# LucaAmbrogioni/Brancher

Measured on AMD Instinct MI355X. Metric: ELBO iters/sec at num_samples=300 per GPU (300-sample-equivalent iterations, whole job), higher is better.
Workload: dtype f32

## Files before the change

brancher_amd/csrc/spec_main.h:

```cpp
#pragma once

namespace bsvi {

#if defined(__HIP_DEVICE_COMPILE__)
#define SPEC_CONST_AS __attribute__((address_space(4)))
#define SPEC_RELOAD_ARGS() asm volatile("" : "+s"(ka))
#else
#define SPEC_CONST_AS
#define SPEC_RELOAD_ARGS()
#endif

#define SPEC_TAB_PTR (4 * SPEC_N_UNIFORM)
#define SPEC_TAB_POS (SPEC_TAB_PTR + SPEC_N_PARAMS + 1)
#define SPEC_TAB_IDX (SPEC_TAB_POS + SPEC_N_POS)
#define SPEC_TAB_MASK (SPEC_TAB_IDX + SPEC_N_POS)

__device__ __forceinline__ void spec_lds_barrier() {
#if defined(__HIP_DEVICE_COMPILE__)
    asm volatile("s_waitcnt lgkmcnt(0)\n\ts_barrier" ::: "memory");
#endif
}

__device__ __noinline__ float spec_utransform_rare(uint32_t t, float x) { return utransform((int)t, x); }
__device__ __noinline__ float spec_utransform_grad_rare(uint32_t t, float x) { return utransform_grad((int)t, x); }
// ... 298 lines not shown
    const uint32_t oid = tid - own_base;
    bool own_fast = false;
#if SPEC_DRAW_OWNERS
    SpecOwn own = {};
#endif
    if (oid < SPEC_N_PARAMS) {
        const uint32_t j0 = TAB[SPEC_TAB_PTR + oid], j1 = TAB[SPEC_TAB_PTR + oid + 1];
        if (j1 - j0 <= 2u) {
            own_fast = true;
#if !SPEC_DRAW_OWNERS
            SpecOwn own;
#endif
            own.n = j1 - j0;
            own.mask = 0;
            own.theta = PS[oid];
            own.s0 = own.s1 = own.s2 = own.st = 0.0f;
            own.p1 = own.p2 = 1.0;
            own.a[0] = own.a[1] = own.b[0] = own.b[1] = 0.0f;
            own.pos[0] = own.pos[1] = own.k[0] = own.k[1] = own.tr[0] = own.tr[1] = 0;
            if (step) {
                own.s0 = PS[SPEC_NP_PAD + oid]; own.s1 = PS[2 * SPEC_NP_PAD + oid];
                own.s2 = PS[3 * SPEC_NP_PAD + oid]; own.st = PS[4 * SPEC_NP_PAD + oid];
                own.mask = TAB[SPEC_TAB_MASK + oid];
                const bsvi_opt_cfg cfg0 = SPEC_A->cfg;
                if (cfg0.kind != BSVI_OPT_SGD && own.st != 0.0f) {
                    own.p1 = pow((double)cfg0.beta1, (double)own.st);
                    own.p2 = pow((double)cfg0.beta2, (double)own.st);
                }
            }
#pragma unroll
            for (uint32_t e = 0; e < 2u; ++e) {
                if (e < own.n) {
                    const uint32_t k = TAB[SPEC_TAB_IDX + j0 + e];
                    own.pos[e] = TAB[SPEC_TAB_POS + j0 + e];
                    own.k[e] = k;
                    own.tr[e] = TAB[4 * k + 1] & 0xFFu;
                    own.a[e] = __uint_as_float(TAB[4 * k + 2]);
                    own.b[e] = __uint_as_float(TAB[4 * k + 3]);
                }
            }
#if !SPEC_DRAW_OWNERS
            spec_own_store(OWN + 5 * oid, own);
#endif
        }
    }

    SPEC_RELOAD_ARGS();
    SpecBody B0;
    B0.n_local = SPEC_A->n_local;
    B0.seed_lo = SPEC_A->seed_lo;
    B0.seed_hi = SPEC_A->seed_hi;
#if SPEC_DIAG
    B0.noise = SPEC_A->noise;
    B0.samples_out = SPEC_A->samples_out;
    B0.noise_out = SPEC_A->noise_out;
    B0.fvalue_out = SPEC_A->fvalue_out;
    B0.f_weight = SPEC_A->f_weight;
    B0.q_weight = SPEC_A->q_weight;
#else
    B0.noise = nullptr; B0.samples_out = nullptr; B0.noise_out = nullptr; B0.fvalue_out = nullptr;
    B0.f_weight = nullptr; B0.q_weight = nullptr;
#endif
    unsigned long long off0 = ((unsigned long long)SPEC_A->offset_hi << 32) | SPEC_A->offset_lo;
    if (const unsigned long long* const offset_dev = SPEC_A->offset_dev) off0 += *offset_dev;
    const uint32_t n_global = SPEC_A->n_global;
    const uint32_t pretraining = SPEC_A->pretraining_iterations;
#if SPEC_ACCUMULATE_CHUNKS
#define SPEC_LOOP_MANY 1
#define SPEC_GEN_OVER 0x7fff0000u
    const unsigned int gen0 = 0;
    if (G > 1 && mode == SPEC_MODE_LOOP && blockIdx.x != 0 &&
        __hip_atomic_load(SPEC_A->ticket + 64, __ATOMIC_RELAXED, __HIP_MEMORY_SCOPE_AGENT) >= SPEC_GEN_OVER) return;
#else
#define SPEC_LOOP_MANY 0
#endif
#if SPEC_EXCHANGE
    uint32_t xseq0 = 0;
    if (const SpecExchange* const xg0 = SPEC_A->xchg) xseq0 = reinterpret_cast<const uint32_t*>(xg0->peer[xg0->rank])[XCHG_CALLS_WORD + 1];
#endif

#if defined(SPEC_DEBUG_STAMPS)
    unsigned long long stamp[12] = {0, 0, 0, 0, 0, 0, 0, 0, 0, 0, 0, 0};
#define SPEC_STAMP(i) if (it == n_it / 2) stamp[i] = __builtin_amdgcn_s_memtime()
    unsigned long long rstamp[6] = {0, 0, 0, 0, 0, 0};
#define SPEC_RSTAMP(i) if (it == n_it / 2) rstamp[i] = __builtin_amdgcn_s_memtime()
#define SPEC_RSTAMP_NEXT() if (it == n_it / 2 + 1u) rstamp[5] = __builtin_amdgcn_s_memtime()
#define SPEC_RSTAMP_WRITE()                                                                                              \
    if (lane == 0u && SPEC_A->loss_slot && n_it > 16u + 8u * SPEC_MAX_WAVES) {                                           \
        asm volatile("s_waitcnt vmcnt(0)" ::: "memory");                                                                 \
        for (int i = 1; i < 6; ++i) SPEC_A->loss_slot[16u + 8u * wave + i] = (float)(rstamp[i] - rstamp[0]);               \
        SPEC_A->loss_slot[16u + 8u * wave] = 1.0f;                                                                       \
    }
#else
#define SPEC_STAMP(i)
#define SPEC_RSTAMP(i)
#define SPEC_RSTAMP_NEXT()
#define SPEC_RSTAMP_WRITE()
#endif
#if SPEC_KEEP_NOISE && !SPEC_DIAG && !SPEC_ACCUMULATE_CHUNKS && !defined(SPEC_DEBUG_NO_DRAW) && !defined(SPEC_NO_EARLY_DRAW)
#define SPEC_EARLY_DRAW 1
    SpecNoise Z;
    bool noise_ready = false;
#else
#define SPEC_EARLY_DRAW 0
#endif
#if SPEC_DRAW_WAVE
    if (draw_service && draw_wave) {
        if (lane == 0u) { RED[8 + 2 * wave] = 0.0f; RED[9 + 2 * wave] = 0.0f; }
        const uint32_t n_draw = W - WSN, k = wave - WSN;
        const uint32_t first = k;
        uint32_t before = 0;
        for (uint32_t j = 0; j < k; ++j) before += (((WSN + j) & 3u) != 1u) ? 1u : 0u;
        const uint32_t second = n_draw + before;
        const bool has_first = first < WSN, has_second = (wave & 3u) != 1u && second < WSN;
        auto draw_for = [&](uint32_t target, unsigned long long offn, SpecNoise& Zd) {
            SpecLane Tn = T;
            Tn.n = target * 64u + lane;
            Tn.active = Tn.n < B0.n_local;
            Tn.nc = Tn.active ? Tn.n : (B0.n_local - 1u);
            Tn.nidx = sample_base + Tn.nc;
            Tn.off_lo = (uint32_t)offn;
            Tn.off_hi = (uint32_t)(offn >> 32);
            Tn.vz = T.vz;
            spec_draw(B0, Tn, Zd);
        };
#if SPEC_DRAW_OWNERS
        (void)has_first; (void)has_second;
        const uint32_t kown = own_wave - WSN, n_other = n_draw - 1u, rest = WSN - 1u;
        const uint32_t j = k < kown ? k : k - 1u, per = rest / n_other, extra = rest % n_other;
        const uint32_t set_a = __builtin_amdgcn_readfirstlane(1u + j * per + (j < extra ? j : extra));
        const uint32_t n_sets = __builtin_amdgcn_readfirstlane(per + (j < extra ? 1u : 0u));
        const bool owners = __builtin_amdgcn_readfirstlane(wave == own_wave ? 1 : 0) != 0;
        for (uint32_t it = 0; it < n_it; ++it) {
            const bool more = it + 1u < n_it, last = !more;
            spec_lds_barrier();
            SPEC_RSTAMP(0);
            SPEC_RSTAMP_NEXT();
            SpecNoise Za, Zb;
            float fac[2] = {0.0f, 0.0f};
            AdamBias bias = {1.0, 1.0, 0.0f, 0.0f};
            if (owners) {
                SPEC_RELOAD_ARGS();
                const bsvi_opt_cfg cfg = SPEC_A->cfg;
#pragma unroll
                for (uint32_t e = 0; e < 2u; ++e) fac[e] = own.b[e] * spec_utransform_grad(own.tr[e], own.theta);
                if (cfg.kind != BSVI_OPT_SGD) bias = optimizer_adam_bias(cfg, own.p1, own.p2);
                if (more) {
                    draw_for(0u, off0 + it + 1u, Za);
                    float* const buf = NZB + (((it + 1u) & 1u) ? WSN * (SPEC_KEEP_NOISE * 64u) : 0u);
#pragma unroll
                    for (uint32_t r = 0; r < SPEC_KEEP_NOISE; ++r) buf[64u * r] = Za.z[r];
                }
            } else if (more) {
                draw_for(set_a, off0 + it + 1u, Za);
                if (n_sets > 1u) draw_for(set_a + 1u, off0 + it + 1u, Zb);
            }
            SPEC_RSTAMP(1);
            spec_lds_barrier();
            SPEC_RSTAMP(2);
            if (owners) {
                SPEC_RELOAD_ARGS();
                float* const out = SPEC_A->out;
                float* const loss_slot = SPEC_A->loss_slot;
                float* const finite_slot = SPEC_A->finite_slot;
                const bsvi_opt_cfg cfg = SPEC_A->cfg;
                float vs = 0.0f, vb = 0.0f;
#pragma unroll
                for (uint32_t w = 0; w < SPEC_MAX_WAVES; ++w) {
                    const float a = RED[8 + 2 * w], b = RED[9 + 2 * w];
                    vs += w < W ? a : 0.0f;
                    vb += w < W ? b : 0.0f;
                }
                float tot[2];
#pragma unroll
                for (uint32_t e = 0; e < 2u; ++e) tot[e] = spec_pos_total(WS, own.pos[e], W);
                const float finite = isfinite(vs) ? 1.0f : 0.0f;
                const float loss = -vs / (float)n_global;
                if (oid == 0u) {
                    if (last) { out[0] = vs; out[1] = vb; out[2] = loss; out[3] = finite; }
                    if (loss_slot) loss_slot[it] = loss;
                    if (finite_slot) finite_slot[it] = finite;
                }
                const float scale = -1.0f / (float)n_global;
                const uint32_t mask_bit = it <= pretraining ? 2u : 1u;
                if (own_fast) {
                    float gsum = 0.0f;
#pragma unroll
                    for (uint32_t e = 0; e < 2u; ++e) {
                        const float term = tot[e] * fac[e];
                        gsum += e < own.n ? term : 0.0f;
                    }
                    const float grad = gsum * scale;
                    SPEC_RSTAMP(3);
                    if (last) out[BSVI_OUT_HEADER + oid] = grad;
                    if (finite != 0.0f && (own.mask & mask_bit)) {
                        if (cfg.kind == BSVI_OPT_SGD) {
                            optimizer_apply(cfg, own.theta, own.s0, own.s1, own.s2, own.st, grad);
                        } else {
                            optimizer_apply_adam_biased(cfg, own.theta, own.s0, own.s1, own.s2, own.st, grad, bias);
                            own.p1 = bias.p1;
                            own.p2 = bias.p2;
                        }
                    }
                    if (last) {
                        float* const params = SPEC_A->params;
                        float* const state = SPEC_A->state;
                        params[oid] = own.theta;
                        if (state) {
                            state[oid] = own.s0;
                            state[(size_t)SPEC_N_PARAMS + oid] = own.s1;
                            state[2 * (size_t)SPEC_N_PARAMS + oid] = own.s2;
                            state[3 * (size_t)SPEC_N_PARAMS + oid] = own.st;
                        }
                    } else {
                        const float g0 = utransform_common(own.tr[0], own.theta);
                        float g1 = g0;
                        if (own.n == 2u && own.tr[1] != own.tr[0]) g1 = utransform_common(own.tr[1], own.theta);
                        if (own.n > 0u) spec_store_uniform(own.k[0], own.a[0] + own.b[0] * g0);
                        if (own.n > 1u) spec_store_uniform(own.k[1], own.a[1] + own.b[1] * g1);
                    }
                }
            } else if (more) {
#pragma unroll
                for (uint32_t r = 0; r < SPEC_KEEP_NOISE; ++r) NZB[set_a * (SPEC_KEEP_NOISE * 64u) + 64u * r] = Za.z[r];
                if (n_sets > 1u) {
#pragma unroll
                    for (uint32_t r = 0; r < SPEC_KEEP_NOISE; ++r) NZB[(set_a + 1u) * (SPEC_KEEP_NOISE * 64u) + 64u * r] = Zb.z[r];
                }
            }
            SPEC_RSTAMP(4);
        }
        SPEC_RSTAMP_WRITE();
        return;
#else
        for (uint32_t it = 0; it < n_it; ++it) {
            const bool more = it + 1u < n_it;
            spec_lds_barrier();
            SPEC_RSTAMP(0);
            SPEC_RSTAMP_NEXT();
            SpecNoise Za;
            if (more && has_first) draw_for(first, off0 + it + 1u, Za);
            SPEC_RSTAMP(1);
            spec_lds_barrier();
            SPEC_RSTAMP(2);
            if (more) {
                if (has_first) {
#pragma unroll
                    for (uint32_t r = 0; r < SPEC_KEEP_NOISE; ++r) NZB[first * (SPEC_KEEP_NOISE * 64u) + 64u * r] = Za.z[r];
                }
                if (has_second) {
                    SpecNoise Zb;
                    draw_for(second, off0 + it + 1u, Zb);
#pragma unroll
                    for (uint32_t r = 0; r < SPEC_KEEP_NOISE; ++r) NZB[second * (SPEC_KEEP_NOISE * 64u) + 64u * r] = Zb.z[r];
                }
            }
            SPEC_RSTAMP(4);
        }
        SPEC_RSTAMP_WRITE();
        return;
#endif
    }
#endif
    for (uint32_t it = 0; it < n_it; ++it) {
        SPEC_STAMP(0);
        float lane_value = 0.0f, lane_bad = 0.0f;
        for (uint32_t chunk = 0; chunk < n_chunks; ++chunk) {
            SpecBody B = B0;
#if SPEC_DIAG
            if (B.noise) B.noise += (size_t)it * SPEC_N_NOISE * B.n_local;
#endif
            T.n = (chunk * G + blockIdx.x) * nthreads + tid;
            T.active = T.n < B.n_local;
            T.nc = T.active ? T.n : (B.n_local - 1u);
            T.nidx = sample_base + T.nc;
            const unsigned long long off = off0 + it;
            T.f = 0.0f;
            T.lq = 0.0f;
#if SPEC_DIAG
            T.gw = B.f_weight ? B.f_weight[T.nc] : 1.0f;
#else
            T.gw = 1.0f;
#endif
            T.off_lo = (uint32_t)off;
            T.off_hi = (uint32_t)(off >> 32);
#if !SPEC_EARLY_DRAW
            SpecNoise Z;
#endif
#if defined(SPEC_DEBUG_NO_DRAW)
            for (uint32_t r = 0; r < (SPEC_KEEP_NOISE ? SPEC_KEEP_NOISE : 1); ++r) Z.z[r] = 0.25f;
#elif SPEC_EARLY_DRAW
#if defined(SPEC_DEBUG_LATE_FREE)
            if (!noise_ready && (!((SPEC_DEBUG_LATE_FREE >> wave) & 1u) || it == 0u)) spec_draw(B, T, Z);
#else
            if (!noise_ready && !draw_wave && !(fed_wave && it > 0u)) spec_draw(B, T, Z);
#endif
#else
            spec_draw(B, T, Z);
#endif
            SPEC_STAMP(1);
            if (chunk == 0) {
                spec_lds_barrier();
                SPEC_RSTAMP(0);
                SPEC_RSTAMP_NEXT();
#if SPEC_ACCUMULATE_CHUNKS
                for (uint32_t k = lane; k < SPEC_WS_CELLS; k += 64u) WSw[k] = 0.0f;
#endif
            }
#if SPEC_DRAW_WAVE
            if (fed_wave && it > 0u) {
#if SPEC_DRAW_OWNERS
// ... 375 lines not shown
```

brancher_amd/csrc/specialize.cpp:

```cpp
#include <hip/hip_runtime.h>
#include <hip/hiprtc.h>
#include <math.h>
#include <stdarg.h>
#include <stdio.h>
#include <stdlib.h>
#include <string.h>
#include <dlfcn.h>
#include <errno.h>
#include <fcntl.h>
#include <link.h>
#include <sys/stat.h>
#include <sys/types.h>
#include <unistd.h>

#include <algorithm>
#include <map>
#include <mutex>
#include <set>
#include <string>
#include <vector>

#include "bsvi.h"
#include "bsvi_internal.h"
#include "spec_args.h"
// ... 442 lines not shown
            }
            int anchor = (int)r;
            if (!samples && reschedule_) {
                int a = -1;
                for (uint32_t sl : rd) {
                    if (sl >= recs[r].temp_base && sl < recs[r].temp_base + recs[r].n_temps) continue;
                    if (def_of[sl] >= 0 && key[def_of[sl]].first > a) a = key[def_of[sl]].first;
                }
                if (a >= 0) anchor = a;
            }
            key[r] = std::make_pair(anchor, (int)r);
            for (uint32_t sl : wr) def_of[sl] = (int)r;
            rorder.push_back(r);
        }
        std::sort(rorder.begin(), rorder.end(), [&](uint32_t x, uint32_t y) { return key[x] > key[y]; });
        std::vector<std::vector<uint32_t>> deferred(recs.size());
        std::vector<int> home(recs.size(), -1);
        if (reschedule_) {
            for (uint32_t r = 0; r < recs.size(); ++r) {
                if (!recs[r].sink) continue;
                std::set<uint32_t> rd, wr;
                slots_of(recs[r], rd, wr);
                int first = -1;
                for (uint32_t sl : rd) {
                    if (sl >= recs[r].temp_base && sl < recs[r].temp_base + recs[r].n_temps) continue;
                    const int dr = def_of[sl];
                    if (dr >= 0 && (uint32_t)dr < r && (first < 0 || key[dr] > key[first])) first = dr;
                }
                if (first >= 0) { home[r] = first; deferred[first].push_back(r); }
            }
        }
        const bool fence = d_.n_code > kFenceAboveCode;
        uint32_t since = 0;
        auto maybe_fence = [&]() { if (fence && ++since >= kFenceEvery) { since = 0; line("asm volatile(\"\" ::: \"memory\"); __builtin_amdgcn_sched_barrier(0);"); } };
        if (two_pass_) line("float f_dead = 0.0f; (void)f_dead;");
        for (uint32_t r = 0; r < recs.size(); ++r) {
            if (home[r] >= 0 && !two_pass_) continue;
            sink_mode_ = home[r] >= 0 ? 1 : 0;
            emit_forward(recs[r]);
            sink_mode_ = 0;
            maybe_fence();
            if (visits_ > kMaxVisits) return;
        }
        if (diag_) line("const float fweight = A.q_weight ? A.q_weight[T.nc] : T.f * T.gw; (void)fweight;");
        else line("const float fweight = T.f; (void)fweight;");
        if (fence) {
            line("asm volatile(\"\" ::: \"memory\");");
            for (uint32_t s0 = 0; s0 < d_.n_slots; s0 += 16) {
                std::string ops;
                for (uint32_t sl = s0; sl < d_.n_slots && sl < s0 + 16; ++sl) ops += fmt("%s\"+v\"(v_%u)", sl == s0 ? "" : ", ", sl);
                line("asm volatile(\"\" : " + ops + ");");
            }
        }
        for (uint32_t r : rorder) {
            sink_mode_ = two_pass_ ? 2 : 0;
            for (uint32_t sidx : deferred[r]) emit_forward(recs[sidx]);
            sink_mode_ = 0;
            emit_reverse(recs[r]);
            maybe_fence();
            if (visits_ > kMaxVisits) return;
        }
        if (diag_) line("if (A.fvalue_out && T.active) { A.fvalue_out[T.n] = T.f; A.fvalue_out[(size_t)A.n_local + T.n] = T.lq; }");
    }
};

}

struct Variant {
    std::string src;
    hipModule_t module = nullptr;
    hipFunction_t fn = nullptr;
    bool failed = false;
    int per_cu = 0;
};

enum { GEOM_ONE = 0, GEOM_MANY = 1 };
struct Geom { uint32_t max_threads = 0, lds_bytes = 0; };

struct Spec {
    uint32_t n_params = 0, n_uniform = 0, n_ugrad = 0, n_obs = 0, n_noise = 0;
    uint32_t n_pos = 0;
    Geom geom[2];
    std::vector<uint32_t> pu_ptr_host, pu_pos_host, pu_idx_host;
    Variant variant[7];
    bool exchange_ok = false;
    void* dev = nullptr;
    unsigned int* tickets = nullptr;
    const uint32_t* pu_ptr = nullptr;
    const uint32_t* pu_pos = nullptr;
    const uint32_t* pu_idx = nullptr;
    uint32_t n_cus = 256;
    bool draw_wave_ok = false;
    uint32_t launch_seq = 0;
    std::mutex mu;
};

static uint32_t many_waves() {
    static const uint32_t w = [] { const char* e = getenv("BSVI_SPEC_MANY_WAVES"); const int v = e ? atoi(e) : 2; return (uint32_t)(v < 2 ? 2 : v > 4 ? 4 : v); }();
    return w;
}
static bool tiled(uint32_t n_pos, int geom) {
    static const bool many_tile = [] { const char* e = getenv("BSVI_SPEC_MANY_TILE"); return !(e && e[0] == '0'); }();
    if (geom == 1  && (!many_tile || many_waves() > 2)) return false;
    return n_pos <= 64;
}
static uint32_t lds_floats(uint32_t n_params, uint32_t n_uniform, uint32_t n_obs, uint32_t n_pos, uint32_t max_threads, int geom) {
    const uint32_t W = max_threads / 64;
    const uint32_t u_pad = (n_uniform + n_obs + 3) / 4 * 4, nu_pad = (n_uniform + 3) / 4 * 4;
    const uint32_t ws_pad = tiled(n_pos, geom) ? (n_pos + 3) / 4 * 4 + 4 : 4 * n_pos + 4;
    const uint32_t np_pad = (n_params + 3) / 4 * 4 + 4, tab = (4 * n_uniform + (2 * n_params + 1) + 2 * n_pos + 3) / 4 * 4 + 4;
    const uint32_t own = 20 * (n_params < max_threads ? n_params : max_threads), scr = 4 * (n_pos + 2) + 4;
    return u_pad + 2 * nu_pad + W * ws_pad + (2 * W + 8) + 5 * np_pad + tab + own + scr + (tiled(n_pos, geom) ? W * 64 * 68 : 0);
}

Spec* create(const bsvi_program_desc& d, std::string& why) {
    if (!d.n_code) { why = "empty program"; return nullptr; }
    Spec* s = new Spec();
    s->n_params = d.n_params; s->n_uniform = d.n_uniform; s->n_ugrad = d.n_uniform_grad; s->n_obs = d.n_obs; s->n_noise = d.n_noise;
    {
        Emitter E(d, false);
        if (!E.run(why)) { delete s; return nullptr; }
        const std::vector<uint32_t>& order = E.order();
        s->n_pos = (uint32_t)order.size();
        std::vector<std::vector<uint32_t>> pos_of(d.n_uniform_grad);
        for (uint32_t p = 0; p < order.size(); ++p) pos_of[order[p]].push_back(p);
        s->pu_ptr_host.assign(1, 0u);
        for (uint32_t i = 0; i < d.n_params; ++i) {
            for (uint32_t j = d.param_uniform_ptr[i]; j < d.param_uniform_ptr[i + 1]; ++j)
                for (uint32_t p : pos_of[d.param_uniform_idx[j]]) { s->pu_pos_host.push_back(p); s->pu_idx_host.push_back(d.param_uniform_idx[j]); }
            s->pu_ptr_host.push_back((uint32_t)s->pu_pos_host.size());
        }
    }
    const uint32_t live = 2 * d.n_slots + (d.n_noise <= kKeepEpsRows ? d.n_noise : 0) + (d.n_uniform_grad <= kAccumulateEntries ? d.n_uniform_grad : 0) + 40;
    auto fit = [&](uint32_t threads, Geom& g) {
        g.max_threads = threads;
        g.lds_bytes = lds_floats(d.n_params, d.n_uniform, d.n_obs, s->n_pos, threads, (int)(&g - s->geom)) * 4u;
        return g.lds_bytes <= 160u * 1024u;
    };
    bool ok = (live <= 232 && fit(512, s->geom[GEOM_ONE])) || fit(256, s->geom[GEOM_ONE]);
    ok = ok && fit(256, s->geom[GEOM_MANY]);
    if (!ok) { why = "the program's tables do not fit LDS"; delete s; return nullptr; }
    bool all_fast = d.n_params <= 64;
    for (uint32_t i = 0; i < d.n_params && all_fast; ++i) all_fast = s->pu_ptr_host[i + 1] - s->pu_ptr_host[i] <= 2;
    s->draw_wave_ok = all_fast && tiled(s->n_pos, GEOM_ONE) && d.n_noise > 0 && d.n_noise <= kKeepEpsRows;
    uint32_t ut_mask = 0;
    for (uint32_t k = 0; k < d.n_uniform; ++k) ut_mask |= 1u << (d.uniform[k].transform & 31u);
    const bool rare_transforms = (ut_mask >> (BSVI_UT_SIGMOID + 1)) != 0;
    for (int gi = 0; gi < 2; ++gi) {
        const Geom& G = s->geom[gi];
        for (int v = 0; v < 2; ++v) {
            Emitter E(d, v == 1);
            if (!E.run(why)) { delete s; return nullptr; }
            std::string src;
            src += "// generated by libbsvi (specialize.cpp) from a model program: do not edit\n";
            src += "#define BSVI_SPECIALIZED 1\n";
            const char* const slp = getenv("BSVI_JIT_SLP");
            if (slp ? slp[0] == '0' : (d.n_code > kFenceAboveCode && d.estimator == BSVI_EST_BLACKBOX))
                src += std::string(kJitOptionMark) + "-fno-slp-vectorize\n";
            const char* const ra = getenv("BSVI_JIT_REGALLOC");
            if (ra ? ra[0] == 'b' : d.n_code > kBasicRegallocAboveCode)
                src += std::string(kJitOptionMark) + "-mllvm\n" + kJitOptionMark + "-vgpr-regalloc=basic\n";
            src += fmt("#define SPEC_N_PARAMS %u\n#define SPEC_N_UNIFORM %u\n#define SPEC_N_UGRAD %u\n#define SPEC_N_OBS %u\n#define SPEC_N_NOISE %u\n",
                       d.n_params, d.n_uniform, d.n_uniform_grad, d.n_obs, d.n_noise);
            src += fmt("#define SPEC_N_POS %u\n", s->n_pos);
            src += fmt("#define SPEC_ESTIMATOR %u\n#define SPEC_MAX_THREADS %u\n#define SPEC_DIAG %d\n", d.estimator, G.max_threads, v);
            src += fmt("#define SPEC_ACCUMULATE_CHUNKS %d\n#define SPEC_TILE %d\n", gi == GEOM_MANY ? 1 : 0, tiled(s->n_pos, gi) ? 1 : 0);
            if (gi == GEOM_MANY && many_waves() > 2) src += fmt("#define SPEC_BOUND_THREADS %u\n", 256u * many_waves());
            src += fmt("#define SPEC_KEEP_NOISE %u\n", E.keeps_noise() ? d.n_noise : 0u);
            src += fmt("#define SPEC_GENERIC_OWNERS %d\n", all_fast ? 0 : 1);
            src += fmt("#define SPEC_RARE_TRANSFORMS %d\n#define SPEC_UT_MASK 0x%xu\n", rare_transforms ? 1 : 0, ut_mask);
            src += "#include \"spec_prelude.h\"\n";
            src += "namespace bsvi {\n";
            src += "__device__ __forceinline__ void spec_draw(const SpecBody& A, const SpecLane& T, SpecNoise& Z) {\n";
            src += "    (void)A; (void)T; (void)Z;\n";
            src += E.draw();
            src += "}\n";
            src += "__device__ __forceinline__ void spec_body(const SpecBody& A, SpecLane& T, const SpecNoise& Z, float* WSw) {\n";
            src += "    (void)Z;\n";
            if (v == 1) src += "    const float* const noise = A.noise;\n";
            src += E.declarations();
            src += E.body();
            src += "}\n}  // namespace bsvi\n";
            src += "#include \"spec_main.h\"\n";
            s->variant[2 * gi + v].src = std::move(src);
        }
    }
    s->variant[4].src = "#define SPEC_WITH_DRAW_WAVE 1\n" + s->variant[0].src;
    s->variant[6].src = "#define SPEC_WITH_DRAW_WAVE 1\n#define SPEC_WITH_DRAW_OWNERS 1\n" + s->variant[0].src;
    s->exchange_ok = true;
    s->variant[5].src = std::string("#define SPEC_WITH_EXCHANGE 1\n") + (s->draw_wave_ok ? "#define SPEC_WITH_DRAW_WAVE 1\n" : "") + s->variant[0].src;
    return s;
}

void destroy(Spec* s) {
    if (!s) return;
    for (Variant& v : s->variant) if (v.module) (void)hipModuleUnload(v.module);
    if (s->dev) (void)hipFree(s->dev);
    delete s;
}

int upload(Spec* s) {
    const size_t n_ptr = s->pu_ptr_host.size(), n_pos = s->pu_pos_host.size();
    const size_t bytes = 512 + (n_ptr + 2 * n_pos) * 4 + 256;
    hipError_t e = hipMalloc(&s->dev, bytes);
    if (e != hipSuccess) return bsvi_fail(BSVI_ERR_HIP, std::string("hipMalloc (specialiser tables): ") + hipGetErrorString(e));
    std::vector<uint32_t> host(128 + n_ptr + 2 * n_pos, 0u);
    std::copy(s->pu_ptr_host.begin(), s->pu_ptr_host.end(), host.begin() + 128);
    std::copy(s->pu_pos_host.begin(), s->pu_pos_host.end(), host.begin() + 128 + n_ptr);
    std::copy(s->pu_idx_host.begin(), s->pu_idx_host.end(), host.begin() + 128 + n_ptr + n_pos);
    e = hipMemset(s->dev, 0, bytes);
    if (e == hipSuccess) e = hipMemcpy(s->dev, host.data(), host.size() * 4, hipMemcpyHostToDevice);
    if (e != hipSuccess) return bsvi_fail(BSVI_ERR_HIP, std::string("specialiser tables: ") + hipGetErrorString(e));
    s->tickets = (unsigned int*)s->dev;
    s->pu_ptr = (const uint32_t*)s->dev + 128;
    s->pu_pos = s->pu_ptr + n_ptr;
    s->pu_idx = s->pu_pos + n_pos;
    int dev = 0, cus = 0;
    if (hipGetDevice(&dev) == hipSuccess && hipDeviceGetAttribute(&cus, hipDeviceAttributeMultiprocessorCount, dev) == hipSuccess && cus > 0)
        s->n_cus = (uint32_t)cus;
    return BSVI_OK;
}

const std::string& source(const Spec* s, int variant) { return s->variant[(variant >= 4 && variant <= 6) ? variant : (variant & 3)].src; }

static const char* kJitOptions[] = {"--offload-arch=gfx950", "-O3", "-std=c++17", "-Xclang", "-target-feature", "-Xclang", "-packed-fp32-ops"};
static const int kJitOptionCount = (int)(sizeof(kJitOptions) / sizeof(kJitOptions[0]));

int compile(const std::string& src, std::vector<char>& code, std::string& log) {
    hiprtcProgram prog = nullptr;
    hiprtcResult r = hiprtcCreateProgram(&prog, src.c_str(), "bsvi_spec.hip", kJitHeaderCount, kJitHeaderTexts, kJitHeaderNames);
    if (r != HIPRTC_SUCCESS) { log = std::string("hiprtcCreateProgram: ") + hiprtcGetErrorString(r); return BSVI_ERR_HIP; }
    std::vector<std::string> extra;
    for (size_t at = src.find(kJitOptionMark); at != std::string::npos; at = src.find(kJitOptionMark, at + 1)) {
        const size_t b = at + strlen(kJitOptionMark), e = src.find('\n', b);
        extra.push_back(src.substr(b, e == std::string::npos ? std::string::npos : e - b));
    }
    std::vector<const char*> opts(kJitOptions, kJitOptions + kJitOptionCount);
    for (const std::string& o : extra) opts.push_back(o.c_str());
    r = hiprtcCompileProgram(prog, (int)opts.size(), opts.data());
    size_t n = 0;
    if (hiprtcGetProgramLogSize(prog, &n) == HIPRTC_SUCCESS && n > 1) {
        log.resize(n);
        (void)hiprtcGetProgramLog(prog, &log[0]);
    }
    if (r != HIPRTC_SUCCESS) {
        log = std::string("hiprtcCompileProgram: ") + hiprtcGetErrorString(r) + "\n" + log;
        (void)hiprtcDestroyProgram(&prog);
        return BSVI_ERR_HIP;
    }
    size_t cs = 0;
    r = hiprtcGetCodeSize(prog, &cs);
    if (r == HIPRTC_SUCCESS) { code.resize(cs); r = hiprtcGetCode(prog, code.data()); }
    (void)hiprtcDestroyProgram(&prog);
    if (r != HIPRTC_SUCCESS) { log = std::string("hiprtcGetCode: ") + hiprtcGetErrorString(r); return BSVI_ERR_HIP; }
    if (const char* dump = getenv("BSVI_JIT_DUMP")) {
        if (FILE* f = fopen(dump, "wb")) { fwrite(code.data(), 1, code.size(), f); fclose(f); }
    }
    return BSVI_OK;
}

static std::mutex g_cache_mu;
static std::map<std::string, std::vector<char>> g_code_cache;

namespace disk_cache {

struct Hash128 { uint64_t a = 0xcbf29ce484222325ull, b = 0x9ae16a3b2f90404full; };
static void feed(Hash128& h, const void* data, size_t n) {
    const unsigned char* p = (const unsigned char*)data;
    for (size_t i = 0; i < n; ++i) {
        h.a = (h.a ^ p[i]) * 0x100000001b3ull;
        h.b = (h.b + p[i] + 0x9e3779b97f4a7c15ull) * 0xff51afd7ed558ccdull;
        h.b ^= h.b >> 29;
    }
}
static void feed(Hash128& h, const std::string& s) { const uint64_t n = s.size(); feed(h, &n, 8); feed(h, s.data(), s.size()); }

static bool enabled() {
    const char* e = getenv("BSVI_JIT_CACHE");
    return !(e && e[0] == '0');
}

static std::string directory() {
    if (const char* d = getenv("BSVI_CACHE_DIR")) if (d[0]) return d;
    if (const char* x = getenv("XDG_CACHE_HOME")) if (x[0]) return std::string(x) + "/brancher_amd/jit";
    if (const char* h = getenv("HOME")) if (h[0]) return std::string(h) + "/.cache/brancher_amd/jit";
    return fmt("/tmp/brancher_amd-%u/jit", (unsigned)getuid());
}

static bool make_dirs(const std::string& path) {
    for (size_t i = 1; i <= path.size(); ++i)
        if (i == path.size() || path[i] == '/') {
            const std::string part = path.substr(0, i);
            if (mkdir(part.c_str(), 0700) != 0 && errno != EEXIST) return false;
        }
    return true;
}

static bool trusted(const std::string& dir) {
    struct stat st;
    if (lstat(dir.c_str(), &st) != 0) return false;
    return S_ISDIR(st.st_mode) && st.st_uid == getuid() && (st.st_mode & (S_IWGRP | S_IWOTH)) == 0;
}

static int identity_cb(struct dl_phdr_info* info, size_t, void* data) {
    const char* name = info->dlpi_name;
    if (!name || !*name) return 0;
// ... 66 lines not shown
    Header H;
    memcpy(H.magic, kMagic, 8);
    H.size = code.size();
    Hash128 h;
    feed(h, code.data(), code.size());
    H.ha = h.a; H.hb = h.b;
    const std::string tmp = dir + "/" + key + fmt(".tmp.%d", (int)getpid());
    const int fd = open(tmp.c_str(), O_WRONLY | O_CREAT | O_EXCL | O_NOFOLLOW | O_CLOEXEC, 0600);
    FILE* f = fd >= 0 ? fdopen(fd, "wb") : nullptr;
    if (!f) { if (fd >= 0) close(fd); return; }
    const bool ok = fwrite(&H, sizeof H, 1, f) == 1 && fwrite(code.data(), 1, code.size(), f) == code.size();
    if (fclose(f) != 0 || !ok || rename(tmp.c_str(), (dir + "/" + key + ".co").c_str()) != 0) (void)remove(tmp.c_str());
}

}

static thread_local int t_last_source = 0;

int obtain(const std::string& text, std::vector<char>& code, std::string& log, int* origin) {
    {
        std::lock_guard<std::mutex> g(g_cache_mu);
        auto it = g_code_cache.find(text);
        if (it != g_code_cache.end()) code = it->second;
    }
    int from = 2;
    if (code.empty()) {
        std::string src = text;
        const bool tuned = getenv("BSVI_SPEC_DEFINES") != nullptr;
        if (tuned) src = std::string(getenv("BSVI_SPEC_DEFINES")) + "\n" + src;
        const bool on_disk = disk_cache::enabled() && !getenv("BSVI_JIT_DUMP");
        const bool lookup = on_disk && disk_cache::identity_resolved(disk_cache::compiler_identity());
        if (lookup && disk_cache::load(disk_cache::key_of(src), code)) {
            from = 3;
        } else {
            const int rc = compile(src, code, log);
            if (rc) return rc;
            from = 1;
            if (on_disk && disk_cache::identity_resolved(disk_cache::compiler_identity())) disk_cache::store(disk_cache::key_of(src), code);
        }
        std::lock_guard<std::mutex> g(g_cache_mu);
        if (!tuned) g_code_cache[text] = code;
    }
    t_last_source = from;
    if (origin) *origin = from;
    return BSVI_OK;
}

int last_origin() { return t_last_source; }
std::string cache_directory() { return disk_cache::enabled() ? disk_cache::directory() : std::string(); }
std::string compiler_identity() { return disk_cache::compiler_identity(); }

static int ensure_compiled(Spec* s, int v) {
    Variant& V = s->variant[v];
    if (V.fn) return BSVI_OK;
    if (V.failed) return BSVI_ERR_UNSUPPORTED;
    std::vector<char> code;
    std::string log;
    if (obtain(V.src, code, log, nullptr)) {
        V.failed = true;
        if (getenv("BSVI_DEBUG")) fprintf(stderr, "bsvi: specialised kernel did not compile:\n%s\n", log.c_str());
        return bsvi_fail(BSVI_ERR_UNSUPPORTED, "specialised kernel did not compile: " + log.substr(0, 400));
    }
    hipError_t e = hipModuleLoadData(&V.module, code.data());
    if (e == hipSuccess) e = hipModuleGetFunction(&V.fn, V.module, "bsvi_spec_kernel");
    if (e != hipSuccess) {
        V.failed = true;
        V.fn = nullptr;
        return bsvi_fail(BSVI_ERR_HIP, std::string("loading the specialised kernel: ") + hipGetErrorString(e));
    }
    return BSVI_OK;
}

struct Geo { uint32_t blocks, threads; int geom; bool draw_wave = false; uint32_t extra_waves = 0; bool draw_owners = false; };
static bool draw_wave() {
    const char* e = getenv("BSVI_SPEC_DRAW_WAVE");
    return !(e && e[0] == '0');
}
static bool draw_service() {
    const char* e = getenv("BSVI_SPEC_DRAW_SERVICE");
    return !(e && e[0] == '0');
}
static bool owner_wave() {
    const char* e = getenv("BSVI_SPEC_OWNER_WAVE");
    return !(e && e[0] == '0');
}
static Geo geo(const Spec* s, uint32_t n_local, int mode = MODE_SUMS, bool exchange = false) {
    const uint32_t waves = (n_local + 63) / 64;
    if (waves <= s->geom[GEOM_ONE].max_threads / 64) {
        const bool extra = mode == MODE_LOOP && s->draw_wave_ok && draw_wave() && waves <= 4 && waves + 1 <= s->geom[GEOM_ONE].max_threads / 64
                           && !s->variant[exchange ? 5 : 4].failed;
        const uint32_t n_service = waves == 4 ? 4u : 3u;
        const bool service = mode == MODE_LOOP && s->draw_wave_ok && draw_wave() && draw_service() && waves >= 4 && waves <= 5
                             && waves + n_service <= s->geom[GEOM_ONE].max_threads / 64 && (size_t)s->n_noise * 64u * waves <= (size_t)n_service * 64u * 68u
                             && !s->variant[exchange ? 5 : 4].failed;
        const uint32_t more = service ? n_service : extra ? 1u : 0u;
        const bool owners = service && (size_t)s->n_noise * 64u * (waves + 1u) <= (size_t)n_service * 64u * 68u;
        return Geo{1, (waves + more) * 64, GEOM_ONE, more != 0u, more, owners};
    }
    const uint32_t threads = s->geom[GEOM_MANY].max_threads;
    uint32_t blocks = (n_local + threads - 1) / threads;
    uint32_t per_cu = many_waves();
    while (per_cu > 1u && s->geom[GEOM_MANY].lds_bytes * per_cu > 160u * 1024u) --per_cu;
    if (blocks > per_cu * s->n_cus) blocks = per_cu * s->n_cus;
    return Geo{blocks, threads, GEOM_MANY};
}

void geometry(const Spec* s, uint32_t n_local, int mode, uint32_t* n_blocks, uint32_t* n_threads, uint32_t* lds_bytes) {
    const Geo g = geo(s, n_local, mode);
    if (n_blocks) *n_blocks = g.blocks;
    if (n_threads) *n_threads = g.threads;
    if (lds_bytes) *lds_bytes = s->geom[g.geom].lds_bytes;
}

size_t workspace_bytes(const Spec* s, uint32_t n_local) {
    const Geo g = geo(s, n_local);
    return ((size_t)g.blocks * (2 + s->n_pos) * 4 + 255) / 256 * 256 + 256;
}

bool applies(const Spec* s, uint32_t n_local, int mode) {
    if (!s || !n_local) return false;
    const char* e = getenv("BSVI_JIT");
    if (e && e[0] == '0') return false;
    const Geo g = geo(s, n_local);
    if (s->variant[2 * g.geom].failed || s->variant[2 * g.geom + 1].failed) return false;
    if (mode == MODE_LOOP && g.blocks != 1) {
        const char* m = getenv("BSVI_SPEC_LOOP_MANY");
        return !(m && m[0] == '0');
    }
    return true;
}

int launch(Spec* s, const bsvi_program* p, const Launch& L) {
    const bsvi_elbo_args* a = L.a;
    if (!a->params_dev && s->n_params) return bsvi_fail(BSVI_ERR_INVALID, "params_dev is null");
    if (!a->obs_dev && s->n_obs) return bsvi_fail(BSVI_ERR_INVALID, "obs_dev is null");
    if (!a->out_dev) return bsvi_fail(BSVI_ERR_INVALID, "out_dev is null");
    if (!a->n_samples_local || !a->n_samples_global) return bsvi_fail(BSVI_ERR_INVALID, "zero samples");
    Geo g = geo(s, a->n_samples_local, L.mode, L.xchg != nullptr);
    int v = 2 * g.geom + ((a->noise_dev || a->samples_out_dev || a->noise_out_dev || a->fvalue_out_dev || a->f_weight_dev || a->q_weight_dev) ? 1 : 0);
    if (L.xchg && !(L.mode == MODE_LOOP && g.blocks == 1 && v == 0 && s->exchange_ok))
        return bsvi_fail(BSVI_ERR_UNSUPPORTED, "the in-loop exchange serves the one-workgroup training loop with Philox noise and no per-sample outputs");
    uint32_t seq;
    {
        std::lock_guard<std::mutex> lock(s->mu);
        if (L.xchg) {
            const int rc5 = ensure_compiled(s, 5);
            if (rc5) return rc5;
            v = 5;
        }
        else if (g.draw_owners && v == 0 && owner_wave()) {
            const int rc6 = ensure_compiled(s, 6);
            if (rc6) return rc6;
            v = 6;
        }
        else if (g.draw_wave && v == 0 && ensure_compiled(s, 4) == BSVI_OK) v = 4;
        else if (g.draw_wave) { g.threads -= 64 * g.extra_waves; g.draw_wave = false; }
        const int rc = ensure_compiled(s, v);
        if (rc) return rc;
        seq = s->launch_seq++;
    }
    if (g.blocks > 1 && !L.workspace) return bsvi_fail(BSVI_ERR_INVALID, "workspace_dev is null");
    SpecArgs A;
    memset(&A, 0, sizeof A);
    A.uniform = p->uniform; A.consts = p->consts;
    A.params = L.params ? L.params : const_cast<float*>(a->params_dev);
    A.obs = a->obs_dev; A.noise = a->noise_dev;
    A.samples_out = a->samples_out_dev; A.noise_out = a->noise_out_dev; A.fvalue_out = a->fvalue_out_dev;
    A.out = a->out_dev;
    A.partials = (float*)L.workspace;
    A.ticket = s->tickets + (seq % 64u);
    A.pu_ptr = s->pu_ptr; A.pu_pos = s->pu_pos; A.pu_idx = s->pu_idx;
    A.state = L.state; A.mask = L.mask; A.mask_first = L.mask_first ? L.mask_first : L.mask;
    A.loss_slot = L.loss_slot; A.finite_slot = L.finite_slot;
    A.n_local = a->n_samples_local; A.n_global = a->n_samples_global; A.sample_base = a->sample_base;
    A.mode = (uint32_t)L.mode;
    A.seed_lo = (uint32_t)a->seed; A.seed_hi = (uint32_t)(a->seed >> 32);
    A.offset_lo = (uint32_t)a->offset; A.offset_hi = (uint32_t)(a->offset >> 32);
    A.offset_dev = (const unsigned long long*)a->offset_dev;
    A.f_weight = a->f_weight_dev; A.q_weight = a->q_weight_dev;
    A.xchg = (const bsvi::SpecExchange*)L.xchg;
    A.n_iterations = L.n_iterations; A.pretraining_iterations = L.pretraining_iterations; A.n_params = s->n_params;
    if (L.cfg) A.cfg = *L.cfg;
    if (g.blocks > 1) {
        int per_cu = s->variant[v].per_cu;
        if (!per_cu) {
            if (hipModuleOccupancyMaxActiveBlocksPerMultiprocessor(&per_cu, s->variant[v].fn, (int)g.threads, 0) != hipSuccess || per_cu <= 0) {
                (void)hipGetLastError();
                per_cu = -1;
            }
            s->variant[v].per_cu = per_cu;
        }
        if (per_cu > 0 && g.blocks > (uint32_t)per_cu * s->n_cus) g.blocks = (uint32_t)per_cu * s->n_cus;
        if (L.mode == MODE_LOOP) {
            hipError_t me = hipMemsetAsync(A.ticket, 0, 4, (hipStream_t)a->stream);
            if (me == hipSuccess) me = hipMemsetAsync(A.ticket + 64, 0, 4, (hipStream_t)a->stream);
            if (me != hipSuccess) return bsvi_fail(BSVI_ERR_HIP, std::string("hipMemsetAsync (loop ticket): ") + hipGetErrorString(me));
        }
    }
    size_t size = sizeof A;
    void* config[] = {HIP_LAUNCH_PARAM_BUFFER_POINTER, &A, HIP_LAUNCH_PARAM_BUFFER_SIZE, &size, HIP_LAUNCH_PARAM_END};
    const hipError_t e = hipModuleLaunchKernel(s->variant[v].fn, g.blocks, 1, 1, g.threads, 1, 1, 0, (hipStream_t)a->stream, nullptr, config);
    if (e != hipSuccess) return bsvi_fail(BSVI_ERR_HIP, std::string("hipModuleLaunchKernel (specialised kernel): ") + hipGetErrorString(e));
    return BSVI_OK;
}

}
```

Baseline: 280,600.

## Move loss epilogue to a noise wave and hoist owner arg loads before barrier

In the owner-wave draw variant, a non-owner draw wave now computes the loss and finite flags and writes them to the loss and finite slots. The owner waves' kernel-argument loads and Adam bias computation are hoisted above the barrier, and they keep only the gradient, optimizer update and uniform stores on the critical path. The owners also read the reductions with vectorized LDS loads. The old epilogue is kept as a new variant 7, selected by the environment flag. This adds source complexity and depends on undisplayed symbols (own_fast, spec_f4) being defined.

```diff
diff --git a/brancher_amd/csrc/spec_main.h b/brancher_amd/csrc/spec_main.h
--- a/brancher_amd/csrc/spec_main.h
+++ b/brancher_amd/csrc/spec_main.h
@@ -404,13 +404,13 @@
 #if defined(SPEC_DEBUG_STAMPS)
     unsigned long long stamp[12] = {0, 0, 0, 0, 0, 0, 0, 0, 0, 0, 0, 0};
 #define SPEC_STAMP(i) if (it == n_it / 2) stamp[i] = __builtin_amdgcn_s_memtime()
-    unsigned long long rstamp[6] = {0, 0, 0, 0, 0, 0};
+    unsigned long long rstamp[8] = {0, 0, 0, 0, 0, 0, 0, 0};
 #define SPEC_RSTAMP(i) if (it == n_it / 2) rstamp[i] = __builtin_amdgcn_s_memtime()
 #define SPEC_RSTAMP_NEXT() if (it == n_it / 2 + 1u) rstamp[5] = __builtin_amdgcn_s_memtime()
 #define SPEC_RSTAMP_WRITE()                                                                                              \
     if (lane == 0u && SPEC_A->loss_slot && n_it > 16u + 8u * SPEC_MAX_WAVES) {                                           \
         asm volatile("s_waitcnt vmcnt(0)" ::: "memory");                                                                 \
-        for (int i = 1; i < 6; ++i) SPEC_A->loss_slot[16u + 8u * wave + i] = (float)(rstamp[i] - rstamp[0]);               \
+        for (int i = 1; i < 8; ++i) SPEC_A->loss_slot[16u + 8u * wave + i] = (float)(rstamp[i] - rstamp[0]);               \
         SPEC_A->loss_slot[16u + 8u * wave] = 1.0f;                                                                       \
     }
 #else
@@ -453,6 +453,9 @@
         const uint32_t set_a = __builtin_amdgcn_readfirstlane(1u + j * per + (j < extra ? j : extra));
         const uint32_t n_sets = __builtin_amdgcn_readfirstlane(per + (j < extra ? 1u : 0u));
         const bool owners = __builtin_amdgcn_readfirstlane(wave == own_wave ? 1 : 0) != 0;
+#if !defined(SPEC_OWNERS_R7_EPILOGUE)
+        const bool loss_wave = __builtin_amdgcn_readfirstlane((!owners && j == 0u) ? 1 : 0) != 0;
+#endif
         for (uint32_t it = 0; it < n_it; ++it) {
             const bool more = it + 1u < n_it, last = !more;
             spec_lds_barrier();
@@ -461,26 +464,49 @@
             SpecNoise Za, Zb;
             float fac[2] = {0.0f, 0.0f};
             AdamBias bias = {1.0, 1.0, 0.0f, 0.0f};
+#if !defined(SPEC_OWNERS_R7_EPILOGUE)
+            float *out = nullptr, *loss_slot = nullptr, *finite_slot = nullptr;
+            bsvi_opt_cfg cfg = {};
+#endif
             if (owners) {
+#if defined(SPEC_OWNERS_R7_EPILOGUE)
                 SPEC_RELOAD_ARGS();
                 const bsvi_opt_cfg cfg = SPEC_A->cfg;
+#endif
 #pragma unroll
                 for (uint32_t e = 0; e < 2u; ++e) fac[e] = own.b[e] * spec_utransform_grad(own.tr[e], own.theta);
+#if defined(SPEC_OWNERS_R7_EPILOGUE)
                 if (cfg.kind != BSVI_OPT_SGD) bias = optimizer_adam_bias(cfg, own.p1, own.p2);
+#endif
                 if (more) {
                     draw_for(0u, off0 + it + 1u, Za);
                     float* const buf = NZB + (((it + 1u) & 1u) ? WSN * (SPEC_KEEP_NOISE * 64u) : 0u);
 #pragma unroll
                     for (uint32_t r = 0; r < SPEC_KEEP_NOISE; ++r) buf[64u * r] = Za.z[r];
                 }
-            } else if (more) {
-                draw_for(set_a, off0 + it + 1u, Za);
-                if (n_sets > 1u) draw_for(set_a + 1u, off0 + it + 1u, Zb);
-            }
+            } else {
+                if (more) {
+                    draw_for(set_a, off0 + it + 1u, Za);
+                    if (n_sets > 1u) draw_for(set_a + 1u, off0 + it + 1u, Zb);
+                }
+            }
+#if !defined(SPEC_OWNERS_R7_EPILOGUE)
+            SPEC_RELOAD_ARGS();
+            if (owners) {
+                out = SPEC_A->out;
+                cfg = SPEC_A->cfg;
+                if (cfg.kind != BSVI_OPT_SGD) bias = optimizer_adam_bias(cfg, own.p1, own.p2);
+            } else if (loss_wave) {
+                out = SPEC_A->out;
+                loss_slot = SPEC_A->loss_slot;
+                finite_slot = SPEC_A->finite_slot;
+            }
+#endif
             SPEC_RSTAMP(1);
             spec_lds_barrier();
             SPEC_RSTAMP(2);
             if (owners) {
+#if defined(SPEC_OWNERS_R7_EPILOGUE)
                 SPEC_RELOAD_ARGS();
                 float* const out = SPEC_A->out;
                 float* const loss_slot = SPEC_A->loss_slot;
@@ -524,6 +550,7 @@
                             own.p2 = bias.p2;
                         }
                     }
+                    SPEC_RSTAMP(6);
                     if (last) {
                         float* const params = SPEC_A->params;
                         float* const state = SPEC_A->state;
@@ -540,15 +567,119 @@
                         if (own.n == 2u && own.tr[1] != own.tr[0]) g1 = utransform_common(own.tr[1], own.theta);
                         if (own.n > 0u) spec_store_uniform(own.k[0], own.a[0] + own.b[0] * g0);
                         if (own.n > 1u) spec_store_uniform(own.k[1], own.a[1] + own.b[1] * g1);
-                    }
-                }
-            } else if (more) {
-#pragma unroll
-                for (uint32_t r = 0; r < SPEC_KEEP_NOISE; ++r) NZB[set_a * (SPEC_KEEP_NOISE * 64u) + 64u * r] = Za.z[r];
-                if (n_sets > 1u) {
-#pragma unroll
-                    for (uint32_t r = 0; r < SPEC_KEEP_NOISE; ++r) NZB[(set_a + 1u) * (SPEC_KEEP_NOISE * 64u) + 64u * r] = Zb.z[r];
-                }
+                        SPEC_RSTAMP(7);
+                    }
+                }
+#else
+                float vs = 0.0f, vb = 0.0f, tot[2] = {0.0f, 0.0f};
+#if SPEC_MAX_WAVES == 8 && SPEC_TILE
+                spec_f4 rq[4], pq[2][2];
+#pragma unroll
+                for (uint32_t q = 0; q < 4u; ++q) rq[q] = *reinterpret_cast<const spec_f4*>(RED + 8 + 4 * q);
+#pragma unroll
+                for (uint32_t e = 0; e < 2u; ++e) {
+#pragma unroll
+                    for (uint32_t q = 0; q < 2u; ++q) {
+                        const float* const c = WS + 4u * q * SPEC_WS_PAD + own.pos[e];
+                        pq[e][q] = spec_f4{c[0], c[SPEC_WS_PAD], c[2 * SPEC_WS_PAD], c[3 * SPEC_WS_PAD]};
+                    }
+                }
+                asm volatile("" : "+v"(rq[0]), "+v"(rq[1]), "+v"(rq[2]), "+v"(rq[3]), "+v"(pq[0][0]), "+v"(pq[0][1]), "+v"(pq[1][0]), "+v"(pq[1][1]));
+#pragma unroll
+                for (uint32_t w = 0; w < SPEC_MAX_WAVES; ++w) {
+                    const float a = rq[w >> 1][2 * (w & 1u)], b = rq[w >> 1][2 * (w & 1u) + 1];
+                    vs += w < W ? a : 0.0f;
+                    vb += w < W ? b : 0.0f;
+                }
+#pragma unroll
+                for (uint32_t e = 0; e < 2u; ++e) {
+#pragma unroll
+                    for (uint32_t w = 0; w < SPEC_MAX_WAVES; ++w) tot[e] += w < W ? pq[e][w >> 2][w & 3u] : 0.0f;
+                }
+#else
+#pragma unroll
+                for (uint32_t w = 0; w < SPEC_MAX_WAVES; ++w) {
+                    const float a = RED[8 + 2 * w], b = RED[9 + 2 * w];
+                    vs += w < W ? a : 0.0f;
+                    vb += w < W ? b : 0.0f;
+                }
+#pragma unroll
+                for (uint32_t e = 0; e < 2u; ++e) tot[e] = spec_pos_total(WS, own.pos[e], W);
+#endif
+                const float finite = isfinite(vs) ? 1.0f : 0.0f;
+                const float scale = -1.0f / (float)n_global;
+                const uint32_t mask_bit = it <= pretraining ? 2u : 1u;
+                float gsum = 0.0f;
+#pragma unroll
+                for (uint32_t e = 0; e < 2u; ++e) {
+                    const float term = tot[e] * fac[e];
+                    gsum += e < own.n ? term : 0.0f;
+                }
+                const float grad = gsum * scale;
+                SPEC_RSTAMP(3);
+                if (own_fast) {
+                    if (finite != 0.0f && (own.mask & mask_bit)) {
+                        if (cfg.kind == BSVI_OPT_SGD) {
+                            optimizer_apply(cfg, own.theta, own.s0, own.s1, own.s2, own.st, grad);
+                        } else {
+                            optimizer_apply_adam_biased(cfg, own.theta, own.s0, own.s1, own.s2, own.st, grad, bias);
+                            own.p1 = bias.p1;
+                            own.p2 = bias.p2;
+                        }
+                    }
+                    SPEC_RSTAMP(6);
+                    if (!last) {
+                        const float g0 = utransform_common(own.tr[0], own.theta);
+                        float g1 = g0;
+                        if (own.n == 2u && own.tr[1] != own.tr[0]) g1 = utransform_common(own.tr[1], own.theta);
+                        if (own.n > 0u) spec_store_uniform(own.k[0], own.a[0] + own.b[0] * g0);
+                        if (own.n > 1u) spec_store_uniform(own.k[1], own.a[1] + own.b[1] * g1);
+                        SPEC_RSTAMP(7);
+                    }
+                }
+                (void)vb;
+                if (last) {
+                    float* const params = SPEC_A->params;
+                    float* const state = SPEC_A->state;
+                    if (own_fast) {
+                        out[BSVI_OUT_HEADER + oid] = grad;
+                        params[oid] = own.theta;
+                        if (state) {
+                            state[oid] = own.s0;
+                            state[(size_t)SPEC_N_PARAMS + oid] = own.s1;
+                            state[2 * (size_t)SPEC_N_PARAMS + oid] = own.s2;
+                            state[3 * (size_t)SPEC_N_PARAMS + oid] = own.st;
+                        }
+                    }
+                }
+#endif
+            } else {
+                if (more) {
+#pragma unroll
+                    for (uint32_t r = 0; r < SPEC_KEEP_NOISE; ++r) NZB[set_a * (SPEC_KEEP_NOISE * 64u) + 64u * r] = Za.z[r];
+                    if (n_sets > 1u) {
+#pragma unroll
+                        for (uint32_t r = 0; r < SPEC_KEEP_NOISE; ++r) NZB[(set_a + 1u) * (SPEC_KEEP_NOISE * 64u) + 64u * r] = Zb.z[r];
+                    }
+                }
+#if !defined(SPEC_OWNERS_R7_EPILOGUE)
+                if (loss_wave) {
+                    float vs = 0.0f, vb = 0.0f;
+#pragma unroll
+                    for (uint32_t w = 0; w < SPEC_MAX_WAVES; ++w) {
+                        const float a = RED[8 + 2 * w], b = RED[9 + 2 * w];
+                        vs += w < W ? a : 0.0f;
+                        vb += w < W ? b : 0.0f;
+                    }
+                    const float finite = isfinite(vs) ? 1.0f : 0.0f;
+                    const float loss = -vs / (float)n_global;
+                    if (lane == 0u) {
+                        if (last) { out[0] = vs; out[1] = vb; out[2] = loss; out[3] = finite; }
+                        if (loss_slot) loss_slot[it] = loss;
+                        if (finite_slot) finite_slot[it] = finite;
+                    }
+                }
+#endif
             }
             SPEC_RSTAMP(4);
         }
diff --git a/brancher_amd/csrc/specialize.cpp b/brancher_amd/csrc/specialize.cpp
--- a/brancher_amd/csrc/specialize.cpp
+++ b/brancher_amd/csrc/specialize.cpp
@@ -548,7 +548,7 @@
     uint32_t n_pos = 0;
     Geom geom[2];
     std::vector<uint32_t> pu_ptr_host, pu_pos_host, pu_idx_host;
-    Variant variant[7];
+    Variant variant[8];
     bool exchange_ok = false;
     void* dev = nullptr;
     unsigned int* tickets = nullptr;
@@ -653,6 +653,7 @@
     }
     s->variant[4].src = "#define SPEC_WITH_DRAW_WAVE 1\n" + s->variant[0].src;
     s->variant[6].src = "#define SPEC_WITH_DRAW_WAVE 1\n#define SPEC_WITH_DRAW_OWNERS 1\n" + s->variant[0].src;
+    s->variant[7].src = "#define SPEC_WITH_DRAW_WAVE 1\n#define SPEC_WITH_DRAW_OWNERS 1\n#define SPEC_OWNERS_R7_EPILOGUE 1\n" + s->variant[0].src;
     s->exchange_ok = true;
     s->variant[5].src = std::string("#define SPEC_WITH_EXCHANGE 1\n") + (s->draw_wave_ok ? "#define SPEC_WITH_DRAW_WAVE 1\n" : "") + s->variant[0].src;
     return s;
@@ -687,7 +688,7 @@
     return BSVI_OK;
 }
 
-const std::string& source(const Spec* s, int variant) { return s->variant[(variant >= 4 && variant <= 6) ? variant : (variant & 3)].src; }
+const std::string& source(const Spec* s, int variant) { return s->variant[(variant >= 4 && variant <= 7) ? variant : (variant & 3)].src; }
 
 static const char* kJitOptions[] = {"--offload-arch=gfx950", "-O3", "-std=c++17", "-Xclang", "-target-feature", "-Xclang", "-packed-fp32-ops"};
 static const int kJitOptionCount = (int)(sizeof(kJitOptions) / sizeof(kJitOptions[0]));
@@ -920,6 +921,10 @@
 }
 static bool owner_wave() {
     const char* e = getenv("BSVI_SPEC_OWNER_WAVE");
+    return !(e && e[0] == '0');
+}
+static bool lean_epilogue() {
+    const char* e = getenv("BSVI_SPEC_LEAN_EPILOGUE");
     return !(e && e[0] == '0');
 }
 static Geo geo(const Spec* s, uint32_t n_local, int mode = MODE_SUMS, bool exchange = false) {
@@ -987,9 +992,10 @@
             v = 5;
         }
         else if (g.draw_owners && v == 0 && owner_wave()) {
-            const int rc6 = ensure_compiled(s, 6);
+            const int vo = lean_epilogue() ? 6 : 7;
+            const int rc6 = ensure_compiled(s, vo);
             if (rc6) return rc6;
-            v = 6;
+            v = vo;
         }
         else if (g.draw_wave && v == 0 && ensure_compiled(s, 4) == BSVI_OK) v = 4;
         else if (g.draw_wave) { g.threads -= 64 * g.extra_waves; g.draw_wave = false; }
```

Result: no change. 282,700, median of 6 (+0.8%).
